# litzendraht/tiny_renderer

Measured on AMD Instinct MI355X. Metric: Mpixels/s shaded (z-test + Phong) at 4096x4096, higher is better.
Workload: dtype f32; 1 GPU; synthetic-sphere-5022, -s phong, 4096x4096; polygons=5022, frames_per_launch=4

## Files before the change

tiny_renderer_amd/csrc/tr_kernels.hip:

```cpp
#include <hip/hip_runtime.h>
#include <hip/hip_ext.h>

#include <type_traits>

#include "tr_kernels.h"
#include "tr_plan.h"
#include "tr_shaders.h"

namespace tr {

namespace {

constexpr int NBY = TILE_H / 8;
constexpr uint32_t NO_WINNER = 0xFFFFFFFFu;
static_assert(NBY == 2 && TILE_H % 4 == 0, "the pixel-pair code assumes two block rows per quadrant");

__device__ __forceinline__ int32_t tile_index(const DevFrame &f, int32_t tx, int32_t ty)
{
    return (ty - f.ty_base) * (int32_t)f.ntx + tx;
}

constexpr uint32_t CHAIN_WAVES = 4;
constexpr uint32_t CHAIN_THREADS = 64 * CHAIN_WAVES;

// ... 477 lines not shown
        if (fs == FS_LIT) want = TR_WPE_LIT_GROUP;
        if (fs == FS_OCCLUSION2) want = TR_WPE_OCCL_GROUP;
        if (shared && want > TR_WPE_SHARED_MAX) want = TR_WPE_SHARED_MAX;
    }
    if (tile_waves == 16) return want >= 6 ? 8 : 4;
    return want;
}
constexpr int lds_rec_bytes_for(int tile_waves, int waves_per_eu, bool shared)
{
    if (tile_waves != 4) return lds_rec_bytes(tile_waves);
    const int per_wg = 160 * 1024 / waves_per_eu / 2560 * 2560;
    const int left = per_wg - TILE_W * TILE_H * 8 - (shared ? 4 * 64 * tile_waves + 4 * tile_waves : 8) - 64;
    const int cap = lds_rec_bytes(4);
    return (left < cap ? left : cap) / 16 * 16;
}

constexpr uint32_t SHARED_MAX_POLYGONS = 1u << 20, SHARED_MAX_SLOTS = 4093u;
#ifndef TR_SCAN_ITEMS
#define TR_SCAN_ITEMS 1
#endif
#ifndef TR_KEY_B64
#define TR_KEY_B64 1
#endif
#ifndef TR_DEPTH_FROM_KEYS
#define TR_DEPTH_FROM_KEYS 1
#endif
constexpr bool SCAN_ITEMS = TR_SCAN_ITEMS != 0;
#ifndef TR_DBG_SKIP
#define TR_DBG_SKIP 0
#endif
__device__ __forceinline__ uint32_t depth_order_bits(float z)
{
    uint32_t b = __float_as_uint(z);
    b = b == 0x80000000u ? 0u : b;
    return (b & 0x80000000u) ? ~b : (b | 0x80000000u);
}

#define TR_TILE_KERNEL_ATTRS \
    __global__ __launch_bounds__(64 * TILE_WAVES) \
        __attribute__((amdgpu_waves_per_eu(tile_waves_per_eu(FS, TILE_WAVES, MODE != 0, SHARED), tile_waves_per_eu(FS, TILE_WAVES, MODE != 0, SHARED))))

template <int FS, int TILE_WAVES, bool SHARED, int MODE>
TR_TILE_KERNEL_ATTRS void k_tile(TileArgs args, const TileArgs *__restrict__ table, uint32_t n_frames)
{
    constexpr bool GROUP = MODE != 0;
    static_assert(TILE_WAVES == 4 || TILE_WAVES == 8 || TILE_WAVES == 16, "a wave covers a 32, 16 or 8 pixel wide column of the tile");
    constexpr int TILE_THREADS = 64 * TILE_WAVES;
    constexpr int QUAD_COLUMN = TILE_W / TILE_WAVES;
    constexpr int WAVES_PER_STRIP = TILE_WAVES / (TILE_W / STRIP);
    constexpr int STRIP_ROWS = TILE_H / WAVES_PER_STRIP;
    static_assert(STRIP_ROWS % 4 == 0, "a shading step covers four rows");
    constexpr bool DEPTH = (FS == FS_DEPTH);
    constexpr int P = (FS == FS_DARBOUX) ? REC_PIECES_LARGE : REC_PIECES_SMALL;
    constexpr int NMAX = lds_rec_bytes_for(TILE_WAVES, tile_waves_per_eu(FS, TILE_WAVES, MODE != 0, SHARED), SHARED) / (P * 16);
    using V2 = std::conditional_t<tile_scalar_pairs(FS), f2s, f2>;

    __shared__ uint2 s_key[TILE_W * TILE_H];
    __shared__ uint4 s_rec[NMAX * P];
    __shared__ uint32_t s_incl[SHARED ? TILE_THREADS : 1];
    __shared__ uint32_t s_wtot[SHARED ? TILE_WAVES : 1];

    const uint32_t n_fr = GROUP ? n_frames : 1u;
    const uint32_t frame_of_group = blockIdx.x % n_fr;
    const TileArgs &a = GROUP ? *(const TileArgs *)(table ? (constant_ptr<TileArgs>)table + frame_of_group
                                                         : (constant_ptr<TileArgs>)__builtin_amdgcn_kernarg_segment_ptr())
                              : args;
    const bool table_lengths = GROUP && table != nullptr;
    const bool fresh = GROUP || a.fresh != 0u;
    const bool st_z = FS == FS_DEPTH || (MODE == 0 ? (a.store & TR_STORE_DEPTH) != 0u : MODE == 1);
    const bool st_c = FS == FS_DEPTH || MODE != 0 || (a.store & TR_STORE_COLOR) != 0u;
    const uint32_t n_tiles = a.frame.ntx * a.frame.nty;
    const uint32_t tid = threadIdx.x;
    __shared__ uint32_t s_stale[EMPTY_CHUNK];
    uint32_t entry = blockIdx.x / n_fr;
    uint32_t list = 0u;
    {
        constant_ptr<uint32_t> lengths = table_lengths ? (constant_ptr<uint32_t>)a.list_len : (constant_ptr<uint32_t>)a.tile_count + n_tiles;
#pragma unroll
        for (int b = 0; b < ORDER_BUCKETS - 1; b++) {
            const uint32_t len = lengths[b];
            if (list == (uint32_t)b && entry >= len) {
                entry -= len;
                list = (uint32_t)b + 1u;
            }
        }
    }
    uint64_t *const stamps = frame_of_group == 0u ? a.stamps : nullptr;
    if (list == (uint32_t)ORDER_EMPTY) {
        constant_ptr<uint32_t> lens = table_lengths ? (constant_ptr<uint32_t>)a.list_len : (constant_ptr<uint32_t>)a.tile_count + n_tiles;
        const uint32_t n_empty = lens[ORDER_EMPTY], first = entry * EMPTY_CHUNK;
        if (first >= n_empty || !fresh) return;
        const uint32_t cnt = min(EMPTY_CHUNK, n_empty - first);
        uint32_t my_tile = 0u;
        bool my_stale = false;
        if (tid < cnt) {
            my_tile = a.order[(size_t)ORDER_EMPTY * n_tiles + first + tid].tile;
            my_stale = st_c && (DEPTH ? a.zclean == nullptr : (a.fbclean == nullptr || gload(a.fbclean + my_tile) == 0u));
            s_stale[tid] = my_stale ? my_tile + 1u : 0u;
        }
        __syncthreads();
        for (uint32_t i = 0; i < cnt; i++) {
            const uint32_t t1 = s_stale[i];
            if (t1 == 0u) continue;
            const uint32_t t = t1 - 1u;
            write_cleared_tile<DEPTH, TILE_THREADS, !GROUP>(a, (int32_t)(t % a.frame.ntx) * TILE_W,
                                      (a.frame.ty_base + (int32_t)(t / a.frame.ntx)) * TILE_H, a.zclean == nullptr);
        }
        if (tid < cnt) {
            if (!DEPTH && my_stale && a.fbclean) a.fbclean[my_tile] = 1u;
            if (a.zclean && st_z) a.zclean[my_tile] = 1u;
        }
        return;
    }
    const WorkItem work = a.order[(size_t)list * n_tiles + entry];
    const uint32_t tile = work.tile;
    uint32_t n = work.count;
    if (tid == 0u) a.tile_count[tile] = 0u;
    if (n == 0u) {
        if (fresh) {
            const bool stale = st_c && (DEPTH || a.fbclean == nullptr || a.fbclean[tile] == 0u);
            __syncthreads();
            if (stale) {
                write_cleared_tile<DEPTH, TILE_THREADS, !GROUP>(a, (int32_t)(tile % a.frame.ntx) * TILE_W,
                                          (a.frame.ty_base + (int32_t)(tile / a.frame.ntx)) * TILE_H, a.zclean == nullptr);
                if (!DEPTH && tid == 0u && a.fbclean) a.fbclean[tile] = 1u;
            }
            if (tid == 0u && a.zclean && st_z) a.zclean[tile] = 1u;
        }
        return;
    }
    const int32_t tx = (int32_t)(tile % a.frame.ntx);
    const int32_t ty = a.frame.ty_base + (int32_t)(tile / a.frame.ntx);
    const int32_t tile_x0 = tx * TILE_W, tile_y0 = ty * TILE_H;
    int32_t W = (int32_t)a.frame.width, H = (int32_t)a.frame.height;
    int32_t band_y0 = a.frame.band_y0, band_y1 = a.frame.band_y1;
    uint32_t aligned4 = a.aligned4;
    uint8_t *fb = a.fb;
    DevTextures tex = a.tex;
    TR_KEEP_SCALAR(W); TR_KEEP_SCALAR(H); TR_KEEP_SCALAR(band_y0); TR_KEEP_SCALAR(band_y1); TR_KEEP_SCALAR(aligned4); TR_KEEP_SCALAR(fb);
    TR_KEEP_SCALAR(tex.packed); TR_KEEP_SCALAR(tex.packed_bpr); TR_KEEP_SCALAR(tex.w[0]); TR_KEEP_SCALAR(tex.h[0]);
    const uint32_t wave = (uint32_t)__builtin_amdgcn_readfirstlane((int)(tid >> 6)), lane = tid & 63u;

    uint64_t t_start = 0, t_staged = 0;
    if (stamps) t_start = wall_clock64();

    float *depth = DEPTH ? a.shadow : a.zbuf;
    const bool zfresh = fresh || (a.zclean && a.zclean[tile] != 0u);
    const int32_t qy0 = tile_y0;
    constexpr uint32_t PREV_TAG = DEPTH ? 0u : 0xFFFFFFFFu;
    const bool shared_tile = SHARED && n >= 2u * (uint32_t)TILE_WAVES && n <= SHARED_MAX_SLOTS;
    const int32_t lx = (int32_t)(lane & 7u), ly = (int32_t)(lane >> 3);
    const uint4 *bin = reinterpret_cast<const uint4 *>(a.bins) + (size_t)work.offset * P;
    const bool resident = n <= (uint32_t)NMAX;

    auto resolve = [&](auto shared_tag) {
        constexpr bool SH = decltype(shared_tag)::value;
        constexpr int QUAD = SH ? TILE_W : QUAD_COLUMN;
        constexpr int NBX = QUAD / 8;
        constexpr int QPIX = QUAD * TILE_H;
        const int32_t qx0 = SH ? tile_x0 : tile_x0 + (int32_t)wave * QUAD;
        uint2 *wkey = SH ? s_key : s_key + wave * QPIX;
        const uint32_t key_lane = SH ? shared_key_slot((uint32_t)lx, (uint32_t)ly) : lane;
        if (SH) {
            for (int b = (int)wave; b < NBX * NBY; b += TILE_WAVES) {
                uint32_t zb = TR_F32_MIN_BITS;
                if (!zfresh) {
                    const int32_t px = qx0 + (b % NBX) * 8 + lx, py = qy0 + (b / NBX) * 8 + ly;
                    if (px < W && py >= band_y0 && py < band_y1)
                        zb = __float_as_uint(gload(depth + ((size_t)py * W + px)));
                }
                wkey[shared_key_slot((uint32_t)((b % NBX) * 8 + lx), (uint32_t)((b / NBX) * 8 + ly))] =
                    make_uint2(PREV_TAG, depth_order_bits(__uint_as_float(zb)));
            }
        } else {
    #pragma unroll
            for (int b = 0; b < NBX * NBY; b++) {
                uint32_t zb = TR_F32_MIN_BITS;
                if (!zfresh) {
                    const int32_t px = qx0 + (b % NBX) * 8 + lx, py = qy0 + (b / NBX) * 8 + ly;
                    if (px < W && py >= band_y0 && py < band_y1)
                        zb = __float_as_uint(gload(depth + ((size_t)py * W + px)));
                }
                wkey[(b << 6) + (lane ^ key_row_swizzle((uint32_t)((int32_t)wave * QUAD + (b % NBX) * 8)))] = make_uint2(zb, 0u);
            }
        }

        for (uint32_t c0 = 0; c0 < n; c0 += NMAX) {
            const uint32_t m = min((uint32_t)NMAX, n - c0);
            if (c0 != 0u) __syncthreads();
            for (uint32_t q = tid; q < m * P; q += (uint32_t)TILE_THREADS) s_rec[q] = gload(bin + ((size_t)c0 * P + q));
            __syncthreads();
            if (stamps && c0 == 0u) t_staged = wall_clock64();

            for (uint32_t j0 = 0; j0 < m; j0 += SH ? 64u * (uint32_t)TILE_WAVES : 64u) {
                const uint32_t jj = SH ? j0 + lane * (uint32_t)TILE_WAVES + wave : j0 + lane;
                uint4 r0 = make_uint4(1u, 0u, 0u, 0u), r1 = make_uint4(0, 0, 0, 0), r2 = r1, r3 = r1;
                uint32_t ry = 0u;
                if (jj < m) {
                    r0 = s_rec[jj * P + 0];
                    r1 = s_rec[jj * P + 1];
                    r2 = s_rec[jj * P + 2];
                    r3 = s_rec[jj * P + 3];
                    ry = s_rec[jj * P + (P - 1)].w;
                }
                const int32_t rbx0 = (int32_t)(r0.x & 0xFFFFu), rbx1 = (int32_t)(r0.x >> 16);
                const int32_t rby0 = (int32_t)(r0.y & 0xFFFFu), rby1 = (int32_t)(r0.y >> 16);
                const PairBox pb = pair_box(rbx0, rbx1, rby0, rby1, tile_x0, qy0);
                const bool some = rbx0 <= rbx1;
                const bool small = SH && SCAN_ITEMS && some && pb.nch <= SCAN_MAX_CHUNKS;
                const uint32_t items = small ? (uint32_t)(__popc(r0.z) + __popc(r0.w)) : 0u;
                uint32_t lmask = (some && !small) ? pair_block_columns(r0.z, r0.w, SHARED && SCAN_ITEMS, pb, tile_x0) : 0u;
                if (!SH) lmask = (lmask >> (NBX * wave)) & ((1u << NBX) - 1u);
                float la0 = __uint_as_float(r1.z), la1 = __uint_as_float(r2.x);
                float lb0 = __uint_as_float(r1.w), lb1 = __uint_as_float(r2.y);
                float lcz = la0 * lb1 - la1 * lb0;
                float lry = __uint_as_float(ry);
                if (lcz < 0.0f) {
                    la0 = -la0; la1 = -la1; lb0 = -lb0; lb1 = -lb1;
                    lcz = -lcz;
                    lry = -lry;
                }
                unsigned long long todo = (TR_DBG_SKIP & 4) ? 0ull : __ballot(lmask != 0u);
                while (todo) {
                    const uint32_t l = (uint32_t)__builtin_ctzll(todo);
                    todo &= todo - 1ull;
                    const uint32_t boxx = (uint32_t)bcast(r0.x, l), boxy = (uint32_t)bcast(r0.y, l);
                    const int32_t bx0 = imax((int32_t)(boxx & 0xFFFFu), qx0), bx1 = imin((int32_t)(boxx >> 16), qx0 + QUAD - 1);
                    const int32_t by0 = imax((int32_t)(boxy & 0xFFFFu), qy0), by1 = imin((int32_t)(boxy >> 16), qy0 + TILE_H - 1);
                    const int32_t x0 = bcast(r1.x, l), y0 = bcast(r1.y, l);
                    const float z0 = __int_as_float(bcast(r2.z, l)), z1 = __int_as_float(bcast(r2.w, l));
                    const float z2 = __int_as_float(bcast(r3.x, l));
                    const uint32_t id = (uint32_t)bcast(r3.y, l);
                    const uint32_t slot1 = SH ? c0 + j0 + l * (uint32_t)TILE_WAVES + wave + 1u : c0 + j0 + l + 1u;
                    uint32_t cols = (uint32_t)bcast(lmask, l);
                    Edge2T<V2> e;
                    e.a0 = splat2v<V2>(__int_as_float(bcast(__float_as_uint(la0), l)));
                    e.a1 = splat2v<V2>(__int_as_float(bcast(__float_as_uint(la1), l)));
                    e.b0 = splat2v<V2>(__int_as_float(bcast(__float_as_uint(lb0), l)));
                    e.b1 = splat2v<V2>(__int_as_float(bcast(__float_as_uint(lb1), l)));
                    const float cz = __int_as_float(bcast(__float_as_uint(lcz), l));
                    e.cz = splat2v<V2>(cz);
                    e.y = splat2v<V2>(__int_as_float(bcast(__float_as_uint(lry), l)));
                    const int32_t pya = qy0 + ly, pyb = qy0 + 8 + ly;
                    const V2 b2 = mk2v<V2>((float)isub(y0, pya), (float)isub(y0, pyb));
                    const bool rowa = pya >= by0 && pya <= by1, rowb = pyb >= by0 && pyb <= by1;
                    const V2 czp = mk2v<V2>(rowa ? cz : -__builtin_inff(), rowb ? cz : -__builtin_inff());
                    while (cols) {
                        const int32_t ib = (int32_t)__builtin_ctz(cols);
                        cols &= cols - 1u;
                        uint2 *slot_a = SH ? wkey + (key_lane ^ ((uint32_t)ib << 3))
                                           : wkey + (((uint32_t)ib << 6) + (lane ^ key_row_swizzle((uint32_t)((int32_t)wave * QUAD + ib * 8))));
                        uint2 *slot_b = slot_a + (SH ? 8 * TILE_W : NBX << 6);
                        const uint2 cur_a = *slot_a, cur_b = *slot_b;
                        const int32_t px = qx0 + ib * 8 + lx;
                        const bool inx = (uint32_t)isub(px, bx0) <= (uint32_t)isub(bx1, bx0);
                        V2 cx, cy;
                        edge_cross2(e, splat2v<V2>((float)isub(x0, px)), b2, cx, cy);
                        const V2 rest = czp - (cx + cy);
                        const bool hita = inx && __builtin_fminf(__builtin_fminf(cx.x, cy.x), rest.x) >= 0.0f;
                        const bool hitb = inx && __builtin_fminf(__builtin_fminf(cx.y, cy.y), rest.y) >= 0.0f;
                        if (SH) {
                            if (hita || hitb) {
                                const Bary2T<V2> bar = barycentric2_for_compare(cx, cy, e);
                                const V2 z = dot3_2(bar.x, bar.y, bar.z, splat2v<V2>(z0), splat2v<V2>(z1), splat2v<V2>(z2));
                                const uint32_t tag = (((SHARED_MAX_POLYGONS - 1u) - id) << 12) | slot1;
                                const unsigned long long ka = ((unsigned long long)depth_order_bits(z.x) << 32) | tag;
                                const unsigned long long kb = ((unsigned long long)depth_order_bits(z.y) << 32) | tag;
                                const unsigned long long ca_ = ((unsigned long long)cur_a.y << 32) | cur_a.x;
                                const unsigned long long cb_ = ((unsigned long long)cur_b.y << 32) | cur_b.x;
                                if (hita && ka > ca_)
                                    __hip_atomic_fetch_max(reinterpret_cast<unsigned long long *>(slot_a), ka, __ATOMIC_RELAXED,
                                                           __HIP_MEMORY_SCOPE_WORKGROUP);
                                if (hitb && kb > cb_)
                                    __hip_atomic_fetch_max(reinterpret_cast<unsigned long long *>(slot_b), kb, __ATOMIC_RELAXED,
                                                           __HIP_MEMORY_SCOPE_WORKGROUP);
                            }
                        } else if (hita || hitb) {
                            const Bary2T<V2> bar = barycentric2_for_compare(cx, cy, e);
                            const V2 z = dot3_2(bar.x, bar.y, bar.z, splat2v<V2>(z0), splat2v<V2>(z1), splat2v<V2>(z2));
                            const float zca = __uint_as_float(cur_a.x), zcb = __uint_as_float(cur_b.x);
                            bool wina = hita && z.x > zca, winb = hitb && z.y > zcb;
                            const bool tiea = hita && z.x == zca, tieb = hitb && z.y == zcb;
                            if (tiea || tieb) {
    #pragma unroll
                                for (int h = 0; h < 2; h++) {
                                    if (!(h == 0 ? tiea : tieb)) continue;
                                    const uint32_t cs = h == 0 ? cur_a.y : cur_b.y;
                                    bool w = DEPTH;
                                    if (cs != 0u) {
                                        const uint32_t cur_id = resident ? s_rec[(cs - 1u) * P + 3].y
                                                                         : gload(bin + ((size_t)(cs - 1u) * P + 3)).y;
                                        w = DEPTH ? id > cur_id : id < cur_id;
                                    }
                                    if (h == 0) wina = w; else winb = w;
                                }
                            }
                            if (wina) *slot_a = make_uint2(__float_as_uint(z.x), slot1);
                            if (winb) *slot_b = make_uint2(__float_as_uint(z.y), slot1);
                        }
                    }
                }

                if (SH && SCAN_ITEMS) {
                    uint32_t incl = items;
    #pragma unroll
                    for (int d = 1; d < 64; d <<= 1) {
                        const uint32_t up = (uint32_t)__shfl_up((int)incl, d, 64);
                        if ((int)lane >= d) incl += up;
                    }
                    if (lane == 63u) s_wtot[wave] = incl;
                    __syncthreads();
                    uint32_t before = 0u, total = 0u;
    #pragma unroll
                    for (int w = 0; w < TILE_WAVES; w++) {
                        const uint32_t t = s_wtot[w];
                        before += (uint32_t)w < wave ? t : 0u;
                        total += t;
                    }
                    total = (uint32_t)__builtin_amdgcn_readfirstlane((int)total);
                    s_incl[tid] = before + incl;
                    __syncthreads();
                    for (uint32_t pass = wave; !(TR_DBG_SKIP & 2) && pass * 64u < total; pass += (uint32_t)TILE_WAVES) {
                        const uint32_t item = pass * 64u + lane;
                        const bool act = item < total;
                        uint32_t lo = 0u, hi = (uint32_t)TILE_THREADS - 1u;
    #pragma unroll
                        for (int i = 0; i < 6 + (TILE_WAVES == 4 ? 2 : TILE_WAVES == 8 ? 3 : 4); i++) {
                            const uint32_t mid = (lo + hi) >> 1;
                            if (s_incl[mid] > item)
                                hi = mid;
                            else
                                lo = mid + 1u;
                        }
                        const uint32_t q = item - (lo ? s_incl[lo - 1u] : 0u);
                        const uint32_t rec = act ? j0 + (lo & 63u) * (uint32_t)TILE_WAVES + (lo >> 6) : 0u;
                        const uint4 *const R = s_rec + mul24(rec, (uint32_t)P);
                        const uint4 q0 = R[0], q1 = R[1], q2 = R[2];
                        const uint2 q3 = *reinterpret_cast<const uint2 *>(R + 3);
                        const float ryv = __uint_as_float(R[P - 1].w);
                        const PairBox ib = pair_box((int32_t)(q0.x & 0xFFFFu), (int32_t)(q0.x >> 16), (int32_t)(q0.y & 0xFFFFu),
                                                    (int32_t)(q0.y >> 16), tile_x0, qy0);
                        uint32_t cell;
                        {
                            const uint32_t nlo = (uint32_t)__popc(q0.z);
                            const bool upper = q >= nlo;
                            uint32_t w = upper ? q0.w : q0.z, k = upper ? q - nlo : q;
                            cell = upper ? 32u : 0u;
    #pragma unroll
                            for (int sh = 16; sh >= 1; sh >>= 1) {
                                const uint32_t below = (uint32_t)__popc(w & ((1u << sh) - 1u));
                                const bool up = k >= below;
                                k -= up ? below : 0u;
                                w = up ? w >> sh : w;
                                cell += up ? (uint32_t)sh : 0u;
                            }
                        }
                        const int32_t py = ib.ay0 + (int32_t)(cell >> 2), xs = ib.xs + 8 * (int32_t)(cell & 3u);
                        const uint32_t first = (uint32_t)imax(isub(ib.ax0, xs), 0) & 7u, last = (uint32_t)imin(isub(ib.ax1, xs), 7) & 7u;
                        const uint32_t inmask = act ? (2u << last) - (1u << first) : 0u;
                        float a0 = __uint_as_float(q1.z), b0 = __uint_as_float(q1.w);
                        float a1 = __uint_as_float(q2.x), b1 = __uint_as_float(q2.y);
                        float cz = a0 * b1 - a1 * b0, yv = ryv;
                        if (cz < 0.0f) {
                            a0 = -a0; a1 = -a1; b0 = -b0; b1 = -b1;
                            cz = -cz;
                            yv = -yv;
                        }
                        const int32_t x0 = (int32_t)q1.x;
                        const float bf = (float)isub((int32_t)q1.y, py);
                        const V2 a1b = splat2v<V2>(a1 * bf), a0b = splat2v<V2>(a0 * bf);
                        Edge2T<V2> e;
                        e.cz = splat2v<V2>(cz);
                        e.y = splat2v<V2>(yv);
                        const V2 z0 = splat2v<V2>(__uint_as_float(q2.z)), z1 = splat2v<V2>(__uint_as_float(q2.w));
                        const V2 z2 = splat2v<V2>(__uint_as_float(q3.x));
                        const uint32_t tag = (((SHARED_MAX_POLYGONS - 1u) - q3.y) << 12) | (c0 + rec + 1u);
                        const uint32_t yrel = (uint32_t)isub(py, qy0) & (uint32_t)(TILE_H - 1);
                        const uint32_t xrel = (uint32_t)isub(xs, qx0) & (uint32_t)(TILE_W - 2);
                        const uint32_t key_row = yrel * (uint32_t)TILE_W, key_sw = (yrel & 7u) << 3;
    #pragma unroll
                        for (int k = 0; k < 4; k++) {
                            const uint32_t kx = (xrel + 2u * k) & (uint32_t)(TILE_W - 1);
                            uint4 *const slot = reinterpret_cast<uint4 *>(wkey + (key_row + (kx ^ key_sw)));
                            const uint4 cur = *slot;
                            const int32_t px = xs + 2 * k;
                            const V2 a2 = mk2v<V2>((float)isub(x0, px), (float)isub(x0, px + 1));
                            const V2 cx = a1b - a2 * splat2v<V2>(b1), cy = a2 * splat2v<V2>(b0) - a0b;
                            const V2 rest = e.cz - (cx + cy);
                            const bool hita = ((inmask >> (2 * k)) & 1u) && __builtin_fminf(__builtin_fminf(cx.x, cy.x), rest.x) >= 0.0f;
                            const bool hitb = ((inmask >> (2 * k + 1)) & 1u) && __builtin_fminf(__builtin_fminf(cx.y, cy.y), rest.y) >= 0.0f;
                            if (hita || hitb) {
                                const Bary2T<V2> bar = barycentric2_for_compare(cx, cy, e);
                                const V2 z = dot3_2(bar.x, bar.y, bar.z, z0, z1, z2);
                                const unsigned long long ka = ((unsigned long long)depth_order_bits(z.x) << 32) | tag;
                                const unsigned long long kb = ((unsigned long long)depth_order_bits(z.y) << 32) | tag;
                                const unsigned long long ca_ = ((unsigned long long)cur.y << 32) | cur.x;
                                const unsigned long long cb_ = ((unsigned long long)cur.w << 32) | cur.z;
                                if (hita && ka > ca_)
                                    __hip_atomic_fetch_max(reinterpret_cast<unsigned long long *>(slot), ka, __ATOMIC_RELAXED,
                                                           __HIP_MEMORY_SCOPE_WORKGROUP);
                                if (hitb && kb > cb_)
                                    __hip_atomic_fetch_max(reinterpret_cast<unsigned long long *>(slot) + 1, kb, __ATOMIC_RELAXED,
                                                           __HIP_MEMORY_SCOPE_WORKGROUP);
                            }
                        }
                    }
                }
            }
        }

    };
    if (shared_tile)
        resolve(std::bool_constant<SHARED>{});
    else
        resolve(std::false_type{});

    uint64_t t_covered = 0;
    if (stamps) t_covered = wall_clock64();

    if (SHARED || TILE_WAVES != TILE_W / STRIP) __syncthreads();
    const int32_t hx = (int32_t)(lane & 31u), hrow = (int32_t)(lane >> 5);
    const uint32_t half_base = lane & 32u;
    const int32_t strip_x = (int32_t)(wave / (uint32_t)WAVES_PER_STRIP) * STRIP;
    const int32_t strip_y = (int32_t)(wave % (uint32_t)WAVES_PER_STRIP) * STRIP_ROWS;
    const int32_t sx0 = tile_x0 + strip_x, sy0 = qy0 + strip_y;
    const int32_t px = sx0 + hx;
    constexpr int NSTEP = STRIP_ROWS / 4;
    float *const depth_strip = depth + ((int64_t)sy0 * W + sx0);
    uint32_t *const winner_strip = (!GROUP && a.winner) ? a.winner + ((int64_t)sy0 * W + sx0) : nullptr;
    uint8_t *const fb_strip = DEPTH ? nullptr : fb + ((int64_t)(H - sy0 - STRIP_ROWS) * W + sx0) * 3;
    const uint32_t Wu = (uint32_t)W, W3 = 3u * (uint32_t)W;
    const bool col_live = px < W;

    auto survivor_slot = [&](uint32_t sx, uint32_t sy, uint32_t &zbits) -> uint32_t {
        if (SHARED && shared_tile) {
            const uint2 key = s_key[shared_key_slot((uint32_t)strip_x + sx, (uint32_t)strip_y + sy)];
            const uint32_t f = key.x & 0xFFFu;
            zbits = (key.y & 0x80000000u) ? key.y ^ 0x80000000u : ~key.y;
            return (f == 0xFFFu) ? 0u : f;
        }
#if TR_KEY_B64
        const uint2 key = s_key[key_slot<QUAD_COLUMN>((uint32_t)strip_x + sx, (uint32_t)strip_y + sy)];
        uint32_t keep = key.x;
        asm volatile("" : "+v"(keep));
        zbits = keep;
        return key.y;
#else
        zbits = 0u;
        return s_key[key_slot<QUAD_COLUMN>((uint32_t)strip_x + sx, (uint32_t)strip_y + sy)].y;
#endif
    };
    auto shade_two = [&](auto in_lds, auto pair_tag, const int32_t (&pxs)[2], const int32_t (&pys)[2], const bool (&won)[2],
                         const uint32_t (&wslot)[2], float (&zout)[2], uint32_t (&rgb)[2], uint32_t (&tri)[2]) -> bool {
        constexpr bool RESIDENT = decltype(in_lds)::value;
        constexpr bool PAIR = decltype(pair_tag)::value;
        bool redo = false;
        constexpr int TOP = P < 6 ? P : 6;
        uint4 qa[TOP], qb[TOP];
        const uint4 *const ra = RESIDENT ? s_rec + mul24(wslot[0], (uint32_t)P) : bin + (size_t)wslot[0] * P;
        const uint4 *const rb = RESIDENT ? s_rec + mul24(wslot[1], (uint32_t)P) : bin + (size_t)wslot[1] * P;
#pragma unroll
        for (int i = 1; i < TOP; i++) {
            qa[i] = RESIDENT ? ra[i] : gload(ra + i);
            qb[i] = RESIDENT ? rb[i] : gload(rb + i);
        }
        const uint32_t rya = P > TOP ? (RESIDENT ? ra[P - 1].w : gload(ra + (P - 1)).w) : qa[TOP - 1].w;
        const uint32_t ryb = P > TOP ? (RESIDENT ? rb[P - 1].w : gload(rb + (P - 1)).w) : qb[TOP - 1].w;
        Edge2T<V2> e;
        e.a0 = mk2v<V2>(__uint_as_float(qa[1].z), __uint_as_float(qb[1].z));
        e.a1 = mk2v<V2>(__uint_as_float(qa[2].x), __uint_as_float(qb[2].x));
        e.b0 = mk2v<V2>(__uint_as_float(qa[1].w), __uint_as_float(qb[1].w));
        e.b1 = mk2v<V2>(__uint_as_float(qa[2].y), __uint_as_float(qb[2].y));
        e.cz = e.a0 * e.b1 - e.a1 * e.b0;
        e.y = mk2v<V2>(__uint_as_float(rya), __uint_as_float(ryb));
        const V2 a2 = mk2v<V2>((float)isub((int32_t)qa[1].x, pxs[0]), (float)isub((int32_t)qb[1].x, pxs[1]));
        const V2 b2 = mk2v<V2>((float)isub((int32_t)qa[1].y, pys[0]), (float)isub((int32_t)qb[1].y, pys[1]));
        V2 cx, cy;
        edge_cross2(e, a2, b2, cx, cy);
        const Bary2T<V2> bar = barycentric2(cx, cy, e);
        const V2 z = dot3_2(bar.x, bar.y, bar.z, mk2v<V2>(__uint_as_float(qa[2].z), __uint_as_float(qb[2].z)),
                            mk2v<V2>(__uint_as_float(qa[2].w), __uint_as_float(qb[2].w)),
                            mk2v<V2>(__uint_as_float(qa[3].x), __uint_as_float(qb[3].x)));
        uint32_t ca = 0u, cb = 0u, ea = 0u, eb = 0u;
        if (!DEPTH && st_c) {
            V2 uu = mk2v<V2>(__uint_as_float(qa[3].z), __uint_as_float(qb[3].z)) * bar.x;
            V2 vv = mk2v<V2>(__uint_as_float(qa[3].w), __uint_as_float(qb[3].w)) * bar.x;
            uu = mk2v<V2>(__uint_as_float(qa[4].x), __uint_as_float(qb[4].x)) * bar.y + uu;
            vv = mk2v<V2>(__uint_as_float(qa[4].y), __uint_as_float(qb[4].y)) * bar.y + vv;
            uu = mk2v<V2>(__uint_as_float(qa[4].z), __uint_as_float(qb[4].z)) * bar.z + uu;
            vv = mk2v<V2>(__uint_as_float(qa[4].w), __uint_as_float(qb[4].w)) * bar.z + vv;
            if (FS == FS_LIT) {
                uint32_t unused1, unused2;
                vec3 unused3;
                fetch_texels<FS>(tex, uu.x, vv.x, ea, ca, unused1, unused2, unused3);
                fetch_texels<FS>(tex, uu.y, vv.y, eb, cb, unused1, unused2, unused3);
            } else if (FS == FS_DEFAULT || FS == FS_PHONG) {
                uint32_t ta, tb, unused1, unused2;
                vec3 unused3;
                fetch_texels<FS>(tex, uu.x, vv.x, ea, ta, unused1, unused2, unused3);
                fetch_texels<FS>(tex, uu.y, vv.y, eb, tb, unused1, unused2, unused3);
                V2 t = mk2v<V2>(__uint_as_float(qa[5].x), __uint_as_float(qb[5].x));
                if (FS == FS_PHONG)
                    t = dot3_2(bar.x, bar.y, bar.z, t, mk2v<V2>(__uint_as_float(qa[5].y), __uint_as_float(qb[5].y)),
                               mk2v<V2>(__uint_as_float(qa[5].z), __uint_as_float(qb[5].z)));
#if TR_BLEND_FAST
                t = mk2v<V2>(blend_weight(t.x), blend_weight(t.y));
#else
                const V2 k = (splat2v<V2>(1.0f) - t) * splat2v<V2>(0.0f);
#endif
#pragma unroll
                for (int ch = 0; ch < 3; ch++) {
#if TR_BLEND_FAST
                    const V2 v = t * mk2v<V2>((float)((ta >> (8 * ch)) & 0xFFu), (float)((tb >> (8 * ch)) & 0xFFu));
#else
                    const V2 v = t * mk2v<V2>((float)((ta >> (8 * ch)) & 0xFFu), (float)((tb >> (8 * ch)) & 0xFFu)) + k;
#endif
                    ca = pack_u8(v.x, (uint32_t)ch, ca);
                    cb = pack_u8(v.y, (uint32_t)ch, cb);
                }
            } else {
                auto closure = [&](const uint4 (&q)[TOP], const uint4 *rec, vec3 b, float u_, float v_, int32_t px_, int32_t py_,
                                   float z_, uint32_t &e_) {
                    float v[VARY_STRIDE];
                    v[0] = __uint_as_float(q[3].z); v[1] = __uint_as_float(q[3].w);
#pragma unroll
                    for (int i = 4; i < P; i++) {
                        const uint4 piece = i < TOP ? q[i] : (RESIDENT ? rec[i] : gload(rec + i));
                        v[4 * i - 14] = __uint_as_float(piece.x); v[4 * i - 13] = __uint_as_float(piece.y);
                        v[4 * i - 12] = __uint_as_float(piece.z); v[4 * i - 11] = __uint_as_float(piece.w);
                    }
                    return fragment_color<FS>(a.u, tex, v, b, u_, v_, (uint32_t)px_, (uint32_t)py_, z_, a.shadow,
                                              (uint32_t)W, (uint32_t)H, e_, a.sclean);
                };
                if constexpr (PAIR) {
                    auto vary2 = [&](int k) -> f2 {
                        const int i = k < 2 ? 3 : (k + 14) / 4, c = k < 2 ? k + 2 : (k + 14) % 4;
                        const uint4 pa = i < TOP ? qa[i] : (RESIDENT ? ra[i] : gload(ra + i)), pb = i < TOP ? qb[i] : (RESIDENT ? rb[i] : gload(rb + i));
                        const uint32_t wa = c == 0 ? pa.x : c == 1 ? pa.y : c == 2 ? pa.z : pa.w;
                        const uint32_t wb = c == 0 ? pb.x : c == 1 ? pb.y : c == 2 ? pb.z : pb.w;
                        return mk2(__uint_as_float(wa), __uint_as_float(wb));
                    };
                    bool bad_a, bad_b;
                    vec3p barp;
                    barp.x = to_f2(bar.x); barp.y = to_f2(bar.y); barp.z = to_f2(bar.z);
                    fragment_color_pair<FS>(a.u, tex, vary2, barp, to_f2(uu), to_f2(vv), ca, cb, ea, eb, bad_a, bad_b);
                    if (__any((bad_a && won[0]) || (bad_b && won[1]))) {
                        redo = true;
                        ea = eb = 0u;
                    }
                } else {
                    ca = closure(qa, ra, make3(bar.x.x, bar.y.x, bar.z.x), uu.x, vv.x, pxs[0], pys[0], z.x, ea);
                    __builtin_amdgcn_sched_barrier(0);
                    cb = closure(qb, rb, make3(bar.x.y, bar.y.y, bar.z.y), uu.y, vv.y, pxs[1], pys[1], z.y, eb);
                }
            }
        }
        uint32_t err = 0u;
        if (won[0]) {
            zout[0] = z.x;
            rgb[0] = ca;
            tri[0] = qa[3].y;
            err |= ea;
        }
        if (won[1]) {
            zout[1] = z.y;
            rgb[1] = cb;
            tri[1] = qb[3].y;
            err |= eb;
        }
        if (err) {
            atomicOr(a.err, err);
            *a.alarm = 1u;
        }
        return redo;
    };

    auto store_pixel = [&](int32_t row, int32_t py_, bool live, bool won, float zv, uint32_t rgbv, uint32_t triv, bool with_winner) {
        const uint32_t zoff = mul24((uint32_t)row, Wu) + (uint32_t)hx;
        const uint32_t coff = mul24((uint32_t)(STRIP_ROWS - 1 - row), W3);
        if (!DEPTH && !fresh && live && !won && st_c) {
            const uint8_t *old = fb_strip + (coff + 3u * (uint32_t)hx);
            rgbv = pack_rgb(gload(old), gload(old + 1), gload(old + 2));
        }
        const bool put = live && (won || zfresh);
        if (put && st_z) gstore(depth_strip + zoff, zv);
        if (!DEPTH && st_c) {
            if (winner_strip && put && with_winner) gstore(winner_strip + zoff, triv);
            if (aligned4) {
                const uint32_t j = (uint32_t)hx;
                const uint32_t p0 = (4u * j) / 3u, o = (4u * j) % 3u;
                const uint32_t c0 = (uint32_t)__shfl((int)rgbv, (int)(half_base + (p0 & 31u)), 64);
                const uint32_t c1 = (uint32_t)__shfl((int)rgbv, (int)(half_base + ((p0 + 1u) & 31u)), 64);
                const uint32_t dw = (c0 >> (8u * o)) | (c1 << (24u - 8u * o));
                const bool row_live = py_ >= band_y0 && py_ < band_y1;
                if (j < 24u && row_live && (sx0 * 3 + (int32_t)(4u * j)) < W * 3)
                    gstore(reinterpret_cast<uint32_t *>(fb_strip + (coff + 4u * j)), dw);
            } else if (put) {
                uint8_t *p = fb_strip + (coff + 3u * (uint32_t)hx);
                gstore(p, (uint8_t)(rgbv & 0xFFu));
                gstore(p + 1, (uint8_t)((rgbv >> 8) & 0xFFu));
                gstore(p + 2, (uint8_t)((rgbv >> 16) & 0xFFu));
            }
        }
    };

    auto shade_steps = [&](auto in_lds, auto pair_tag, uint32_t step_mask) -> uint32_t {
    uint32_t redo = 0u;
#pragma unroll 1
    for (int32_t sstep = 0; sstep < NSTEP; sstep++) {
        if (!((step_mask >> sstep) & 1u)) continue;
        int32_t row[2], py[2];
        bool live[2], won[2];
        uint32_t wslot[2], zkey[2];
#pragma unroll
        for (int u = 0; u < 2; u++) {
            row[u] = sstep * 4 + u * 2 + hrow;
            py[u] = sy0 + row[u];
            live[u] = col_live && py[u] >= band_y0 && py[u] < band_y1;
            const uint32_t s1 = survivor_slot((uint32_t)hx, (uint32_t)row[u], zkey[u]);
            won[u] = live[u] && s1 != 0u;
            wslot[u] = won[u] ? s1 - 1u : 0u;
        }
        uint32_t tri[2] = { NO_WINNER, NO_WINNER }, rgb[2] = { 0u, 0u };
        float zout[2] = { bits_f32(TR_F32_MIN_BITS), bits_f32(TR_F32_MIN_BITS) };
        bool from_keys = false;
        if (DEPTH && TR_DEPTH_FROM_KEYS && TR_KEY_B64) {
            from_keys = !__any((won[0] && (zkey[0] << 1) == 0u) || (won[1] && (zkey[1] << 1) == 0u));
            if (from_keys) {
                if (won[0]) zout[0] = __uint_as_float(zkey[0]);
                if (won[1]) zout[1] = __uint_as_float(zkey[1]);
            }
        }
        if (!(TR_DBG_SKIP & 1) && !from_keys && __any(won[0] || won[1])) {
            const int32_t pxs[2] = { px, px };
            if (shade_two(in_lds, pair_tag, pxs, py, won, wslot, zout, rgb, tri)) redo |= 1u << sstep;
        }
#pragma unroll
        for (int u = 0; u < 2; u++) store_pixel(row[u], py[u], live[u], won[u], zout[u], rgb[u], tri[u], true);
    }
    return redo;
    };

    constexpr uint32_t ALL_STEPS = (1u << NSTEP) - 1u;
    constexpr bool HAS_PAIR = has_pair_closure(FS);
    uint32_t redo;
    if (resident)
        redo = shade_steps(std::true_type{}, std::bool_constant<HAS_PAIR>{}, ALL_STEPS);
    else
        redo = shade_steps(std::false_type{}, std::bool_constant<HAS_PAIR>{}, ALL_STEPS);
    if (HAS_PAIR && redo != 0u) {
        if (resident)
            shade_steps(std::true_type{}, std::false_type{}, redo);
        else
            shade_steps(std::false_type{}, std::false_type{}, redo);
    }

    if (a.zclean && tid == 0u && st_z) a.zclean[tile] = 0u;
    if (!DEPTH && a.fbclean && tid == 0u && st_c) a.fbclean[tile] = 0u;

    if (stamps) {
        __syncthreads();
        if (tid == 0u) {
            stamps[8u * tile + 0u] = t_start;
            stamps[8u * tile + 1u] = wall_clock64();
            stamps[8u * tile + 2u] = n;
            stamps[8u * tile + 3u] = __smid();
            stamps[8u * tile + 4u] = t_staged;
            stamps[8u * tile + 5u] = t_covered;
        }
    }
}


__global__ __launch_bounds__(256) void k_materialize_depth(float *zbuf, uint32_t *zclean, DevFrame frame)
{
    const uint32_t t = blockIdx.x;
    if (zclean[t] == 0u) return;
    const int32_t x0 = (int32_t)(t % frame.ntx) * TILE_W, y0 = (frame.ty_base + (int32_t)(t / frame.ntx)) * TILE_H;
    for (uint32_t p = threadIdx.x; p < (uint32_t)(TILE_W * TILE_H); p += 256u) {
        const int32_t y = y0 + (int32_t)(p / TILE_W), x = x0 + (int32_t)(p % TILE_W);
        if (x < (int32_t)frame.width && y >= frame.band_y0 && y < frame.band_y1)
            zbuf[(size_t)y * frame.width + x] = bits_f32(TR_F32_MIN_BITS);
    }
    __syncthreads();
    if (threadIdx.x == 0u) zclean[t] = 0u;
}

__global__ __launch_bounds__(256) void k_depth_view(const float *src, uint8_t *dst, uint32_t W, uint32_t H)
{
    const size_t n = (size_t)W * H;
    const size_t stride = (size_t)gridDim.x * blockDim.x;
    for (size_t i = (size_t)blockIdx.x * blockDim.x + threadIdx.x; i < n; i += stride) {
        const uint32_t y = (uint32_t)(i / W), x = (uint32_t)(i % W);
        const uint8_t v = (uint8_t)f32_to_u8(src[i]);
        uint8_t *p = dst + ((size_t)(H - 1u - y) * W + x) * 3;
        p[0] = v;
        p[1] = v;
        p[2] = v;
    }
}

__global__ __launch_bounds__(256) void k_read_back(const uint8_t *__restrict__ fb, uint8_t *__restrict__ host,
                                                   const uint32_t *__restrict__ fb_clean, uint32_t *host_clean, DevFrame frame)
{
    const uint32_t t = blockIdx.x;
    const bool zeros = fb_clean[t] != 0u;
    const bool host_zeros = host_clean[t] != 0u;
    __syncthreads();
    if (zeros && host_zeros) return;
    const int32_t W = (int32_t)frame.width, H = (int32_t)frame.height;
    const int32_t x0 = (int32_t)(t % frame.ntx) * TILE_W, y0 = (frame.ty_base + (int32_t)(t / frame.ntx)) * TILE_H;
    for (uint32_t c = threadIdx.x; c < (uint32_t)TILE_H * 24u; c += 256u) {
        const int32_t y = y0 + (int32_t)(c / 24u);
        const int32_t xb = x0 * 3 + (int32_t)(c % 24u) * 16;
        if (xb < W * 3 && y >= frame.band_y0 && y < frame.band_y1) {
            const size_t at = (size_t)(H - 1 - y) * W * 3 + xb;
            const uint4 v = zeros ? make_uint4(0u, 0u, 0u, 0u) : *reinterpret_cast<const uint4 *>(fb + at);
            *reinterpret_cast<uint4 *>(host + at) = v;
        }
    }
    if (threadIdx.x == 0u) host_clean[t] = zeros ? 1u : 0u;
}

__global__ __launch_bounds__(256) void k_push_tiles(const uint8_t *__restrict__ fb, uint8_t *__restrict__ peer,
                                                    const uint32_t *__restrict__ fb_clean, uint32_t *remote_clean, DevFrame frame,
                                                    const uint32_t *poisoned, unsigned long long *bytes)
{
    __shared__ uint32_t s_poisoned;
    if (threadIdx.x == 0u) s_poisoned = __hip_atomic_load(poisoned, __ATOMIC_RELAXED, __HIP_MEMORY_SCOPE_SYSTEM);
    const uint32_t t = blockIdx.x;
    const bool zeros = fb_clean[t] != 0u;
    const bool remote_zeros = remote_clean[t] != 0u;
    __syncthreads();
    if (s_poisoned != 0u) return;
    if (zeros && remote_zeros) return;
    const int32_t W = (int32_t)frame.width, H = (int32_t)frame.height;
    const int32_t x0 = (int32_t)(t % frame.ntx) * TILE_W, y0 = (frame.ty_base + (int32_t)(t / frame.ntx)) * TILE_H;
    uint32_t pieces = 0;
    for (uint32_t c = threadIdx.x; c < (uint32_t)TILE_H * 24u; c += 256u) {
        const int32_t y = y0 + (int32_t)(c / 24u);
        const int32_t xb = x0 * 3 + (int32_t)(c % 24u) * 16;
        if (xb < W * 3 && y >= frame.band_y0 && y < frame.band_y1) {
            const size_t at = (size_t)(H - 1 - y) * W * 3 + xb;
            const uint4 v = zeros ? make_uint4(0u, 0u, 0u, 0u) : *reinterpret_cast<const uint4 *>(fb + at);
            *reinterpret_cast<uint4 *>(peer + at) = v;
            pieces++;
        }
    }
    if (pieces) atomicAdd(bytes, (unsigned long long)pieces * 16ull);
    if (threadIdx.x == 0u) remote_clean[t] = zeros ? 1u : 0u;
}

__global__ __launch_bounds__(256) void k_selftest(const float *x, const float *d, uint32_t n, uint32_t *out_u32,
                                                  int32_t *out_i32, uint32_t *out_u8, float *out_div,
                                                  float *out_div_ref)
{
    const uint32_t i = blockIdx.x * blockDim.x + threadIdx.x;
    if (i >= n) return;
    out_u32[i] = f32_to_u32(x[i]);
    out_i32[i] = f32_to_i32(x[i]);
    out_u8[i] = f32_to_u8(x[i]);
    out_div[i] = div_by(x[i], recip_of(d[i]));
    out_div_ref[i] = x[i] / d[i];
}

__global__ __launch_bounds__(256) void k_selftest_shadow(const float *plain, const float *stale, const uint32_t *sclean,
                                                         uint32_t W, uint32_t H, const float *x, const float *y, uint32_t n,
                                                         uint32_t *out_plain, uint32_t *out_flagged, uint32_t *err_plain,
                                                         uint32_t *err_flagged)
{
    const uint32_t i = blockIdx.x * blockDim.x + threadIdx.x;
    if (i >= n) return;
    uint32_t e0 = 0u, e1 = 0u;
    const float a = shadow_fetch(plain, nullptr, W, H, make3(x[i], y[i], 0.0f), e0);
    const float b = shadow_fetch(stale, sclean, W, H, make3(x[i], y[i], 0.0f), e1);
    out_plain[i] = __float_as_uint(a);
    out_flagged[i] = __float_as_uint(b);
    err_plain[i] = e0;
    err_flagged[i] = e1;
}

__global__ __launch_bounds__(256) void k_selftest_unary(int which, uint32_t first, uint64_t count,
                                                        unsigned long long *n_bad, uint32_t *bad_bits)
{
    const uint64_t stride = (uint64_t)gridDim.x * blockDim.x;
    for (uint64_t i = (uint64_t)blockIdx.x * blockDim.x + threadIdx.x; i < count; i += stride) {
        const float x = __uint_as_float(first + (uint32_t)i);
        float got, want;
        if (which == 2) {
            const uint32_t into = 0xA5C3E17Bu, b = (uint32_t)(i & 3u);
            const uint32_t g0 = pack_u8(x, b, into), w0 = (into & ~(0xFFu << (8u * b))) | (f32_to_u8(x) << (8u * b));
// ... 338 lines not shown
```

Measured before the change: 222,800 Mpixels/s.

## Load rasterizer triangle records via scalar loads and hoist per-lane address math

```diff
diff --git a/tiny_renderer_amd/csrc/tr_kernels.hip b/tiny_renderer_amd/csrc/tr_kernels.hip
--- a/tiny_renderer_amd/csrc/tr_kernels.hip
+++ b/tiny_renderer_amd/csrc/tr_kernels.hip
@@ -653,6 +653,9 @@
     const int32_t lx = (int32_t)(lane & 7u), ly = (int32_t)(lane >> 3);
     const uint4 *bin = reinterpret_cast<const uint4 *>(a.bins) + (size_t)work.offset * P;
     const bool resident = n <= (uint32_t)NMAX;
+    const uint64_t bin_addr = reinterpret_cast<uint64_t>(bin);
+    const constant_ptr<uint32_t> bin_s = (constant_ptr<uint32_t>)(((uint64_t)(uint32_t)__builtin_amdgcn_readfirstlane((int)(uint32_t)(bin_addr >> 32)) << 32) |
+                                                            (uint32_t)__builtin_amdgcn_readfirstlane((int)(uint32_t)bin_addr));
 
     auto resolve = [&](auto shared_tag) {
         constexpr bool SH = decltype(shared_tag)::value;
@@ -695,14 +698,11 @@
 
             for (uint32_t j0 = 0; j0 < m; j0 += SH ? 64u * (uint32_t)TILE_WAVES : 64u) {
                 const uint32_t jj = SH ? j0 + lane * (uint32_t)TILE_WAVES + wave : j0 + lane;
-                uint4 r0 = make_uint4(1u, 0u, 0u, 0u), r1 = make_uint4(0, 0, 0, 0), r2 = r1, r3 = r1;
-                uint32_t ry = 0u;
+                uint4 r0 = make_uint4(1u, 0u, 0u, 0u), r1 = make_uint4(0, 0, 0, 0), r2 = r1;
                 if (jj < m) {
                     r0 = s_rec[jj * P + 0];
                     r1 = s_rec[jj * P + 1];
                     r2 = s_rec[jj * P + 2];
-                    r3 = s_rec[jj * P + 3];
-                    ry = s_rec[jj * P + (P - 1)].w;
                 }
                 const int32_t rbx0 = (int32_t)(r0.x & 0xFFFFu), rbx1 = (int32_t)(r0.x >> 16);
                 const int32_t rby0 = (int32_t)(r0.y & 0xFFFFu), rby1 = (int32_t)(r0.y >> 16);
@@ -712,36 +712,35 @@
                 const uint32_t items = small ? (uint32_t)(__popc(r0.z) + __popc(r0.w)) : 0u;
                 uint32_t lmask = (some && !small) ? pair_block_columns(r0.z, r0.w, SHARED && SCAN_ITEMS, pb, tile_x0) : 0u;
                 if (!SH) lmask = (lmask >> (NBX * wave)) & ((1u << NBX) - 1u);
-                float la0 = __uint_as_float(r1.z), la1 = __uint_as_float(r2.x);
-                float lb0 = __uint_as_float(r1.w), lb1 = __uint_as_float(r2.y);
-                float lcz = la0 * lb1 - la1 * lb0;
-                float lry = __uint_as_float(ry);
-                if (lcz < 0.0f) {
-                    la0 = -la0; la1 = -la1; lb0 = -lb0; lb1 = -lb1;
-                    lcz = -lcz;
-                    lry = -lry;
-                }
+                const float lcz_raw = __uint_as_float(r1.z) * __uint_as_float(r2.y) - __uint_as_float(r2.x) * __uint_as_float(r1.w);
+                const unsigned long long flip = __ballot(lcz_raw < 0.0f);
+                const float lcz = lcz_raw < 0.0f ? -lcz_raw : lcz_raw;
                 unsigned long long todo = (TR_DBG_SKIP & 4) ? 0ull : __ballot(lmask != 0u);
                 while (todo) {
                     const uint32_t l = (uint32_t)__builtin_ctzll(todo);
                     todo &= todo - 1ull;
-                    const uint32_t boxx = (uint32_t)bcast(r0.x, l), boxy = (uint32_t)bcast(r0.y, l);
+                    const uint32_t slot1 = SH ? c0 + j0 + l * (uint32_t)TILE_WAVES + wave + 1u : c0 + j0 + l + 1u;
+                    const constant_ptr<uint32_t> rec = bin_s + (slot1 - 1u) * (uint32_t)(4 * P);
+                    const uint4 g0 = make_uint4(rec[0], rec[1], 0u, 0u), g1 = make_uint4(rec[4], rec[5], rec[6], rec[7]);
+                    const uint4 g2 = make_uint4(rec[8], rec[9], rec[10], rec[11]), g3 = make_uint4(rec[12], rec[13], 0u, 0u);
+                    const uint32_t gry = rec[4 * P - 1];
+                    const uint32_t sgn = ((uint32_t)(flip >> l) & 1u) << 31;
+                    const uint32_t boxx = g0.x, boxy = g0.y;
                     const int32_t bx0 = imax((int32_t)(boxx & 0xFFFFu), qx0), bx1 = imin((int32_t)(boxx >> 16), qx0 + QUAD - 1);
                     const int32_t by0 = imax((int32_t)(boxy & 0xFFFFu), qy0), by1 = imin((int32_t)(boxy >> 16), qy0 + TILE_H - 1);
-                    const int32_t x0 = bcast(r1.x, l), y0 = bcast(r1.y, l);
-                    const float z0 = __int_as_float(bcast(r2.z, l)), z1 = __int_as_float(bcast(r2.w, l));
-                    const float z2 = __int_as_float(bcast(r3.x, l));
-                    const uint32_t id = (uint32_t)bcast(r3.y, l);
-                    const uint32_t slot1 = SH ? c0 + j0 + l * (uint32_t)TILE_WAVES + wave + 1u : c0 + j0 + l + 1u;
+                    const int32_t x0 = (int32_t)g1.x, y0 = (int32_t)g1.y;
+                    const float z0 = __uint_as_float(g2.z), z1 = __uint_as_float(g2.w);
+                    const float z2 = __uint_as_float(g3.x);
+                    const uint32_t id = g3.y;
                     uint32_t cols = (uint32_t)bcast(lmask, l);
                     Edge2T<V2> e;
-                    e.a0 = splat2v<V2>(__int_as_float(bcast(__float_as_uint(la0), l)));
-                    e.a1 = splat2v<V2>(__int_as_float(bcast(__float_as_uint(la1), l)));
-                    e.b0 = splat2v<V2>(__int_as_float(bcast(__float_as_uint(lb0), l)));
-                    e.b1 = splat2v<V2>(__int_as_float(bcast(__float_as_uint(lb1), l)));
+                    e.a0 = splat2v<V2>(__uint_as_float(g1.z ^ sgn));
+                    e.a1 = splat2v<V2>(__uint_as_float(g2.x ^ sgn));
+                    e.b0 = splat2v<V2>(__uint_as_float(g1.w ^ sgn));
+                    e.b1 = splat2v<V2>(__uint_as_float(g2.y ^ sgn));
                     const float cz = __int_as_float(bcast(__float_as_uint(lcz), l));
                     e.cz = splat2v<V2>(cz);
-                    e.y = splat2v<V2>(__int_as_float(bcast(__float_as_uint(lry), l)));
+                    e.y = splat2v<V2>(__uint_as_float(gry ^ sgn));
                     const int32_t pya = qy0 + ly, pyb = qy0 + 8 + ly;
                     const V2 b2 = mk2v<V2>((float)isub(y0, pya), (float)isub(y0, pyb));
                     const bool rowa = pya >= by0 && pya <= by1, rowb = pyb >= by0 && pyb <= by1;
@@ -932,23 +931,32 @@
     uint8_t *const fb_strip = DEPTH ? nullptr : fb + ((int64_t)(H - sy0 - STRIP_ROWS) * W + sx0) * 3;
     const uint32_t Wu = (uint32_t)W, W3 = 3u * (uint32_t)W;
     const bool col_live = px < W;
-
-    auto survivor_slot = [&](uint32_t sx, uint32_t sy, uint32_t &zbits) -> uint32_t {
+    const uint32_t key_lane = key_slot<QUAD_COLUMN>((uint32_t)strip_x + (uint32_t)hx, (uint32_t)hrow);
+    const uint32_t zlane = mul24((uint32_t)hrow, Wu) + (uint32_t)hx;
+    const uint32_t clane = mul24(1u - (uint32_t)hrow, W3);
+    const uint32_t cj = (uint32_t)hx, cp0 = (4u * cj) / 3u, co = (4u * cj) % 3u;
+    const int32_t perm0 = (int32_t)((half_base + (cp0 & 31u)) << 2), perm1 = (int32_t)((half_base + ((cp0 + 1u) & 31u)) << 2);
+    const uint32_t csh0 = 8u * co, csh1 = 24u - 8u * co;
+    const bool cdw_live = cj < 24u && (sx0 * 3 + (int32_t)(4u * cj)) < W * 3;
+
+    auto survivor_slot = [&](uint32_t r0, uint32_t &zbits) -> uint32_t {
         if (SHARED && shared_tile) {
-            const uint2 key = s_key[shared_key_slot((uint32_t)strip_x + sx, (uint32_t)strip_y + sy)];
+            const uint2 key = s_key[shared_key_slot((uint32_t)strip_x + (uint32_t)hx, (uint32_t)strip_y + r0 + (uint32_t)hrow)];
             const uint32_t f = key.x & 0xFFFu;
             zbits = (key.y & 0x80000000u) ? key.y ^ 0x80000000u : ~key.y;
             return (f == 0xFFFu) ? 0u : f;
         }
+        const uint32_t ry = (uint32_t)strip_y + r0;
+        const uint32_t slot = (key_lane ^ ((ry & 7u) << 3)) + (((ry >> 3) * (uint32_t)(QUAD_COLUMN / 8)) << 6);
 #if TR_KEY_B64
-        const uint2 key = s_key[key_slot<QUAD_COLUMN>((uint32_t)strip_x + sx, (uint32_t)strip_y + sy)];
+        const uint2 key = s_key[slot];
         uint32_t keep = key.x;
         asm volatile("" : "+v"(keep));
         zbits = keep;
         return key.y;
 #else
         zbits = 0u;
-        return s_key[key_slot<QUAD_COLUMN>((uint32_t)strip_x + sx, (uint32_t)strip_y + sy)].y;
+        return s_key[slot].y;
 #endif
     };
     auto shade_two = [&](auto in_lds, auto pair_tag, const int32_t (&pxs)[2], const int32_t (&pys)[2], const bool (&won)[2],
@@ -958,8 +966,8 @@
         bool redo = false;
         constexpr int TOP = P < 6 ? P : 6;
         uint4 qa[TOP], qb[TOP];
-        const uint4 *const ra = RESIDENT ? s_rec + mul24(wslot[0], (uint32_t)P) : bin + (size_t)wslot[0] * P;
-        const uint4 *const rb = RESIDENT ? s_rec + mul24(wslot[1], (uint32_t)P) : bin + (size_t)wslot[1] * P;
+        const uint4 *const ra = RESIDENT ? s_rec + ((int32_t)mul24(wslot[0], (uint32_t)P) - P) : bin + (size_t)wslot[0] * P;
+        const uint4 *const rb = RESIDENT ? s_rec + ((int32_t)mul24(wslot[1], (uint32_t)P) - P) : bin + (size_t)wslot[1] * P;
 #pragma unroll
         for (int i = 1; i < TOP; i++) {
             qa[i] = RESIDENT ? ra[i] : gload(ra + i);
@@ -1076,28 +1084,25 @@
         return redo;
     };
 
-    auto store_pixel = [&](int32_t row, int32_t py_, bool live, bool won, float zv, uint32_t rgbv, uint32_t triv, bool with_winner) {
-        const uint32_t zoff = mul24((uint32_t)row, Wu) + (uint32_t)hx;
-        const uint32_t coff = mul24((uint32_t)(STRIP_ROWS - 1 - row), W3);
+    auto store_pixel = [&](uint32_t r0, bool row_live, bool live, bool won, float zv, uint32_t rgbv,
+                           uint32_t triv, bool with_winner) {
+        uint8_t *const fb_row = DEPTH ? nullptr : fb_strip + (int64_t)((int32_t)(STRIP_ROWS - 2) - (int32_t)r0) * (int64_t)W3;
         if (!DEPTH && !fresh && live && !won && st_c) {
-            const uint8_t *old = fb_strip + (coff + 3u * (uint32_t)hx);
+            const uint8_t *old = fb_row + (clane + 3u * (uint32_t)hx);
             rgbv = pack_rgb(gload(old), gload(old + 1), gload(old + 2));
         }
         const bool put = live && (won || zfresh);
-        if (put && st_z) gstore(depth_strip + zoff, zv);
+        if (put && st_z) gstore(depth_strip + (int64_t)r0 * W + zlane, zv);
         if (!DEPTH && st_c) {
-            if (winner_strip && put && with_winner) gstore(winner_strip + zoff, triv);
+            if (winner_strip && put && with_winner) gstore(winner_strip + (int64_t)r0 * W + zlane, triv);
             if (aligned4) {
-                const uint32_t j = (uint32_t)hx;
-                const uint32_t p0 = (4u * j) / 3u, o = (4u * j) % 3u;
-                const uint32_t c0 = (uint32_t)__shfl((int)rgbv, (int)(half_base + (p0 & 31u)), 64);
-                const uint32_t c1 = (uint32_t)__shfl((int)rgbv, (int)(half_base + ((p0 + 1u) & 31u)), 64);
-                const uint32_t dw = (c0 >> (8u * o)) | (c1 << (24u - 8u * o));
-                const bool row_live = py_ >= band_y0 && py_ < band_y1;
-                if (j < 24u && row_live && (sx0 * 3 + (int32_t)(4u * j)) < W * 3)
-                    gstore(reinterpret_cast<uint32_t *>(fb_strip + (coff + 4u * j)), dw);
+                const uint32_t c0 = (uint32_t)__builtin_amdgcn_ds_bpermute(perm0, (int)rgbv);
+                const uint32_t c1 = (uint32_t)__builtin_amdgcn_ds_bpermute(perm1, (int)rgbv);
+                const uint32_t dw = (c0 >> csh0) | (c1 << csh1);
+                if (cdw_live && row_live)
+                    gstore(reinterpret_cast<uint32_t *>(fb_row + (clane + 4u * cj)), dw);
             } else if (put) {
-                uint8_t *p = fb_strip + (coff + 3u * (uint32_t)hx);
+                uint8_t *p = fb_row + (clane + 3u * (uint32_t)hx);
                 gstore(p, (uint8_t)(rgbv & 0xFFu));
                 gstore(p + 1, (uint8_t)((rgbv >> 8) & 0xFFu));
                 gstore(p + 2, (uint8_t)((rgbv >> 16) & 0xFFu));
@@ -1106,21 +1111,23 @@
     };
 
     auto shade_steps = [&](auto in_lds, auto pair_tag, uint32_t step_mask) -> uint32_t {
+    constexpr bool RESIDENT = decltype(in_lds)::value;
     uint32_t redo = 0u;
 #pragma unroll 1
     for (int32_t sstep = 0; sstep < NSTEP; sstep++) {
         if (!((step_mask >> sstep) & 1u)) continue;
-        int32_t row[2], py[2];
-        bool live[2], won[2];
+        int32_t py[2];
+        bool row_live[2], live[2], won[2];
         uint32_t wslot[2], zkey[2];
 #pragma unroll
         for (int u = 0; u < 2; u++) {
-            row[u] = sstep * 4 + u * 2 + hrow;
-            py[u] = sy0 + row[u];
-            live[u] = col_live && py[u] >= band_y0 && py[u] < band_y1;
-            const uint32_t s1 = survivor_slot((uint32_t)hx, (uint32_t)row[u], zkey[u]);
+            const uint32_t r0 = (uint32_t)(sstep * 4 + u * 2);
+            py[u] = sy0 + (int32_t)r0 + hrow;
+            row_live[u] = py[u] >= band_y0 && py[u] < band_y1;
+            live[u] = col_live && row_live[u];
+            const uint32_t s1 = survivor_slot(r0, zkey[u]);
             won[u] = live[u] && s1 != 0u;
-            wslot[u] = won[u] ? s1 - 1u : 0u;
+            wslot[u] = RESIDENT ? s1 : (won[u] ? s1 - 1u : 0u);
         }
         uint32_t tri[2] = { NO_WINNER, NO_WINNER }, rgb[2] = { 0u, 0u };
         float zout[2] = { bits_f32(TR_F32_MIN_BITS), bits_f32(TR_F32_MIN_BITS) };
@@ -1137,7 +1144,8 @@
             if (shade_two(in_lds, pair_tag, pxs, py, won, wslot, zout, rgb, tri)) redo |= 1u << sstep;
         }
 #pragma unroll
-        for (int u = 0; u < 2; u++) store_pixel(row[u], py[u], live[u], won[u], zout[u], rgb[u], tri[u], true);
+        for (int u = 0; u < 2; u++)
+            store_pixel((uint32_t)(sstep * 4 + u * 2), row_live[u], live[u], won[u], zout[u], rgb[u], tri[u], true);
     }
     return redo;
     };
```

New measurement: 236,900 Mpixels/s (median of 6 runs). +6.4%, better.
